# vbronetskyi/nclt-slam-project

Measured on AMD Instinct MI355X. Metric: relocalization frames/sec @640x480, 10k-landmark DB; Hamming-match HBM GB/s, higher is better.
Workload: dtype u8; 1 GPU; 640x480 BGR frames, 10000-record landmark DB (640000 descriptors, rows=fixed64), global relocalization tick per frame: ORB(500) + whole-DB mutual Hamming scan + top-25 PnP-RANSAC(200); frames resident in HBM, every frame's 96-byte result record written to pinned host memory by the tick's last kernel; distinct_frames=32, preroll_steps=20, streams=4, records=10000, descriptors=640000, parallelism=frames sharded across ranks, database replicated, no collective

## Files before the change

nclt-slam-project_amd/csrc/reloc_ctx.hip:

```cpp
#include <stdarg.h>
#include <stdlib.h>

#include "reloc_internal.h"

static thread_local char g_err[512] = "";

void reloc_set_error(const char *fmt, ...)
{
    va_list ap;
    va_start(ap, fmt);
    vsnprintf(g_err, sizeof(g_err), fmt, ap);
    va_end(ap);
}

RELOC_API const char *reloc_last_error(void) { return g_err; }

RELOC_API int reloc_device_count(void)
{
    int n = 0;
    if (hipGetDeviceCount(&n) != hipSuccess) return 0;
    return n;
}

template <typename T>
static int dalloc(T **p, int64_t count)
{
    HIP_TRY(hipMalloc((void **)p, (size_t)(count > 0 ? count : 1) * sizeof(T)));
    return 0;
}

static int ctx_alloc(reloc_ctx *c)
{
    int rc = 0;
    const int64_t mf = c->max_feat;
    int64_t pyr = 0;
    for (int l = 0; l < NLEV; ++l) {
        double s = pow(RELOC_ORB_SCALE_FACTOR, (double)l);
        int64_t w = (int64_t)(c->max_w / s) + 2, h = (int64_t)(c->max_h / s) + 2;
        pyr += ((w + 63) / 64 * 64) * h + 256;
    }
    c->pyr_bytes = pyr;
    rc |= dalloc(&c->pyr, pyr);
    rc |= dalloc(&c->blur, pyr);
    rc |= dalloc(&c->nms, pyr);
    rc |= dalloc(&c->rz_tab, (int64_t)NLEV * 2 * 2 * (c->max_w > c->max_h ? c->max_w : c->max_h));
    rc |= dalloc((char **)&c->pyr_tiles, (int64_t)((c->max_w + 15) / 16) * ((c->max_h + 15) / 16) * 128);
    rc |= dalloc(&c->hist, NLEV * 256);
    rc |= dalloc(&c->cand_cnt, NLEV);
    rc |= dalloc(&c->cand_key, (int64_t)NLEV * RELOC_ORB_STAGE1_CAP);
    rc |= dalloc(&c->cand_resp, (int64_t)NLEV * RELOC_ORB_STAGE1_CAP);
    rc |= dalloc(&c->kp_cnt, NLEV);
    rc |= dalloc(&c->kp_key, (int64_t)NLEV * RELOC_ORB_STAGE1_CAP);
    rc |= dalloc(&c->kp_resp, (int64_t)NLEV * RELOC_ORB_STAGE1_CAP);
    rc |= dalloc(&c->f_xy, mf * 2);
    rc |= dalloc(&c->f_size, mf);
    rc |= dalloc(&c->f_angle, mf);
    rc |= dalloc(&c->f_resp, mf);
    rc |= dalloc(&c->f_oct, mf);
    rc |= dalloc(&c->f_desc, mf * 32);
    rc |= dalloc(&c->f_count, 1);
    rc |= dalloc(&c->frame_img, (int64_t)c->max_w * c->max_h * 3);
    rc |= dalloc((char **)&c->orb_const, 1024);
    rc |= dalloc(&c->dbg_cut, NLEV);
    rc |= dalloc(&c->cand_ids, MAX_CAND);
    rc |= dalloc(&c->cand_n, 1);
    rc |= dalloc(&c->m_qidx, (int64_t)MAX_CAND * MAX_REC_ROWS);
    rc |= dalloc(&c->m_tidx, (int64_t)MAX_CAND * MAX_REC_ROWS);
    rc |= dalloc(&c->m_dist, (int64_t)MAX_CAND * MAX_REC_ROWS);
    rc |= dalloc(&c->m_n, MAX_CAND);
    rc |= dalloc(&c->p_obj, (int64_t)MAX_CAND * MAX_REC_ROWS * 3);
    rc |= dalloc(&c->p_img, (int64_t)MAX_CAND * MAX_REC_ROWS * 2);
    rc |= dalloc(&c->p_Rt, (int64_t)MAX_CAND * MAX_HYP * 12);
    rc |= dalloc(&c->p_cnt, (int64_t)MAX_CAND * MAX_HYP);
    rc |= dalloc(&c->p_inl, (int64_t)MAX_CAND * MAX_REC_ROWS);
    rc |= dalloc(&c->p_out, MAX_CAND);
    rc |= dalloc(&c->tick_res, 1);
    if (hipHostMalloc((void **)&c->tick_res_host, sizeof(TickResult), hipHostMallocDefault) != hipSuccess) {
        reloc_set_error("hipHostMalloc(result record) failed");
        c->tick_res_host = nullptr;
        rc |= RELOC_E_HIP;
    } else memset(c->tick_res_host, 0, sizeof(TickResult));
    rc |= dalloc(&c->accum_res, 1);
    rc |= dalloc(&c->tick_flags, 4);
    rc |= dalloc(&c->scan_ticket, (8 * 8 + 1) * 32);
    if (rc == 0 && hipMemset(c->scan_ticket, 0, (8 * 8 + 1) * 32 * 4) != hipSuccess) rc = RELOC_E_HIP;
    return rc;
}

int g_reloc_live_contexts = 0;

RELOC_API reloc_ctx *reloc_create(int device, int max_w, int max_h, int max_feat)
{
    int n = 0;
    if (hipGetDeviceCount(&n) != hipSuccess || n <= 0) {
        reloc_set_error("no HIP device available (libreloc_hip has no CPU fallback)");
        return nullptr;
    }
    if (device < 0 || device >= n || max_w < 64 || max_h < 64 || max_feat < 64) {
        reloc_set_error("reloc_create: bad arguments (device %d of %d, %dx%d, max_feat %d)", device, n,
                        max_w, max_h, max_feat);
        return nullptr;
    }
    if (hipSetDevice(device) != hipSuccess) {
        reloc_set_error("hipSetDevice(%d) failed", device);
        return nullptr;
    }
    reloc_ctx *c = new reloc_ctx();
    __atomic_add_fetch(&g_reloc_live_contexts, 1, __ATOMIC_RELAXED);
    c->device = device;
    c->max_w = max_w;
    c->max_h = max_h;
    c->max_feat = max_feat;
    hipDeviceProp_t prop;
    if (hipGetDeviceProperties(&prop, device) == hipSuccess) c->num_cu = prop.multiProcessorCount;
    if (hipStreamCreateWithFlags(&c->own_stream, hipStreamNonBlocking) != hipSuccess ||
        hipEventCreate(&c->t0) != hipSuccess || hipEventCreate(&c->t1) != hipSuccess) {
        reloc_set_error("stream/event creation failed");
        __atomic_sub_fetch(&g_reloc_live_contexts, 1, __ATOMIC_RELAXED);
        delete c;
        return nullptr;
    }
    c->stream = c->own_stream;
    c->prm.nfeatures = 500;
    c->prm.max_candidates = RELOC_MAX_CANDIDATES;
    c->prm.min_matches = RELOC_MIN_MATCHES;
    c->prm.min_inliers = RELOC_MIN_INLIERS;
    c->prm.ransac_iterations = RELOC_RANSAC_ITERATIONS;
    c->prm.global_max_candidates = RELOC_GLOBAL_MAX_CANDIDATES;
    c->prm.global_min_inliers = RELOC_GLOBAL_MIN_INLIERS;
    c->prm.accum_min_kpts = RELOC_ACCUM_MIN_KPTS;
    c->prm.candidate_radius_m = RELOC_CANDIDATE_RADIUS_M;
    c->prm.heading_tol_deg = RELOC_HEADING_TOL_DEG;
    c->prm.reproj_max_px = RELOC_REPROJ_MAX_PX;
    c->prm.ransac_reproj_px = RELOC_RANSAC_REPROJ_PX;
    c->prm.ransac_confidence = RELOC_RANSAC_CONFIDENCE;
    c->prm.consistency_m = RELOC_CONSISTENCY_M;
    c->prm.global_reproj_max_px = RELOC_GLOBAL_REPROJ_MAX_PX;
    c->prm.accum_min_dist_m = RELOC_ACCUM_MIN_DIST_M;
    c->prm.accum_depth_min_m = RELOC_ACCUM_DEPTH_MIN_M;
    c->prm.accum_depth_max_m = RELOC_ACCUM_DEPTH_MAX_M;
    c->prm.gray_coeff_bits = RELOC_GRAY_DEFAULT_BITS;
    c->prm.reserved0 = 0;
    if (const char *dev = getenv("RELOC_DEV"); dev && dev[0] == '1' && dev[1] == 0) {
        if (const char *e = getenv("RELOC_SCAN_GENS")) c->scan_gens = atoi(e);
        if (const char *e = getenv("RELOC_LOCAL_TWO_STAGE")) c->local_two_stage = atoi(e) != 0;
    }
    if (ctx_alloc(c) != 0) {
        reloc_destroy(c);
        return nullptr;
    }
    return c;
}

RELOC_API void reloc_destroy(reloc_ctx *c)
{
    if (!c) return;
    (void)hipSetDevice(c->device);
    if (c->stream) (void)hipStreamSynchronize(c->stream);
    db_arrays_drop(c->db_share, c->db_desc, c->db_pts3d, c->db_kp2d, c->db_off, c->db_pose, c->db_xy_heading);
    void *ptrs[] = {c->pyr, c->blur, c->nms, c->rz_tab, c->pyr_tiles, c->hist, c->cand_cnt, c->cand_key, c->cand_resp,
                    c->kp_cnt, c->kp_key, c->kp_resp, c->f_xy, c->f_size, c->f_angle, c->f_resp, c->f_oct,
                    c->f_desc, c->f_count, c->frame_img, c->orb_const, c->dbg_cut, c->db_counts, c->topk_part, c->cand_ids, c->cand_n, c->m_qidx,
                    c->m_tidx, c->m_dist, c->m_n, c->p_obj, c->p_img, c->p_Rt, c->p_cnt, c->p_inl,
                    c->p_out, c->tick_res, c->accum_res, c->tick_flags, c->scan_ticket, c->clahe_plane, c->clahe_lut,
                    c->rect_xy };
    for (void *p : ptrs)
        if (p) (void)hipFree(p);
    if (c->tick_res_host) (void)hipHostFree(c->tick_res_host);
    {
        DbArena &a = c->db_slot[1 - c->db_sel];
        db_arrays_drop(a.share, a.desc, a.pts3d, a.kp2d, a.off, a.pose, a.xy_heading);
        if (a.counts) (void)hipFree(a.counts);
        if (a.topk_part) (void)hipFree(a.topk_part);
    }
    for (int i = 0; i < 8; ++i)
        if (c->scratch[i]) (void)hipFree(c->scratch[i]);
    for (int k = 0; k < RELOC_PROF_N; ++k)
        if (c->prof[k].init)
            for (int i = 0; i < RELOC_PROF_RING; ++i) {
                (void)hipEventDestroy(c->prof[k].a[i]);
                (void)hipEventDestroy(c->prof[k].b[i]);
            }
    if (c->t0) (void)hipEventDestroy(c->t0);
    if (c->t1) (void)hipEventDestroy(c->t1);
    if (c->own_stream) (void)hipStreamDestroy(c->own_stream);
    __atomic_sub_fetch(&g_reloc_live_contexts, 1, __ATOMIC_RELAXED);
    delete c;
}

RELOC_API int reloc_get_params(reloc_ctx *c, reloc_params *out)
{
    ARG_CHECK_CTX(c, out, "reloc_get_params");
    *out = c->prm;
    return RELOC_OK;
}

RELOC_API int reloc_set_params(reloc_ctx *c, const reloc_params *p)
{
    ARG_CHECK_CTX(c, p, "reloc_set_params");
// ... 181 lines not shown
```

nclt-slam-project_amd/csrc/reloc_orb.hip:

```cpp
#include <math.h>

#include "../../include/reloc_orb_pattern.h"
#include "reloc_internal.h"

typedef uint32_t u32;

constexpr int HARRIS_CHUNK = 1024;
static_assert(HARRIS_CHUNK == 1024, "k_harris reads one dword per thread");

struct OrbTable {
    OrbLevel lev[NLEV];
    int fast_tile_base[NLEV + 1];
    int blur_tile_base[NLEV + 1];
    int flat_base[NLEV + 1];
    int rz_off[NLEV][4];
};

__constant__ signed char c_pattern[RELOC_ORB_NTESTS * 4];
__constant__ int c_umax[16] = {15, 15, 15, 15, 14, 14, 14, 13, 13, 12, 11, 10, 9, 8, 6, 3};
__constant__ signed char c_ring_dx[16] = {0, 1, 2, 3, 3, 3, 2, 1, 0, -1, -2, -3, -3, -3, -2, -1};
__constant__ signed char c_ring_dy[16] = {3, 3, 2, 1, 0, -1, -2, -3, -3, -3, -2, -1, 0, 1, 2, 3};

__device__ __forceinline__ int find_level(const int *base, int id)
{
    int l = 0;
#pragma unroll
    for (int k = 1; k < NLEV; ++k) l += id >= base[k];
    return l;
}

__device__ __forceinline__ int reflect101(int p, int n)
{
    if (n == 1) return 0;
    while (p < 0 || p >= n) {
        if (p < 0) p = -p;
        if (p >= n) p = 2 * n - 2 - p;
    }
    return p;
}

__device__ __forceinline__ int gray_fixed(int b, int g, int r, int flags)
{
    const bool c15 = flags & RELOC_GRAY_FLAG_15BIT;
    const int cb = c15 ? RELOC_GRAY15_CB : RELOC_GRAY_CB, cg = c15 ? RELOC_GRAY15_CG : RELOC_GRAY_CG, cr = c15 ? RELOC_GRAY15_CR : RELOC_GRAY_CR;
    const int sh = c15 ? RELOC_GRAY15_SHIFT : RELOC_GRAY_SHIFT;
    return (b * cb + g * cg + r * cr + (1 << (sh - 1))) >> sh;
}
static inline int gray_flags(const reloc_ctx *ctx, int order)
{
    return (order & 1) | (ctx->prm.gray_coeff_bits == RELOC_GRAY15_SHIFT ? RELOC_GRAY_FLAG_15BIT : 0);
}
__global__ __launch_bounds__(256) void k_gray_plain(const uint8_t *__restrict__ src, int w, int h, int sstride, int order_rgb,
                                                    uint8_t *__restrict__ dst)
{
    const int x = blockIdx.x * 256 + threadIdx.x, y = blockIdx.y;
    if (x >= w) return;
    const uint8_t *s = src + (size_t)y * sstride + 3 * x;
    const int c0 = s[0], c1 = s[1], c2 = s[2];
    const int b = (order_rgb & 1) ? c2 : c0, r = (order_rgb & 1) ? c0 : c2;
    dst[(size_t)y * w + x] = (uint8_t)gray_fixed(b, c1, r, order_rgb);
}

#ifndef PYR_TW
#define PYR_TW 64
#define PYR_TH 32
#endif
constexpr int PT_W = PYR_TW, PT_H = PYR_TH;
struct PyrTile {
    uint16_t o[NLEV][4];
    uint16_t n[NLEV][4];
};
static_assert(sizeof(PyrTile) == 128, "PyrTile is read as 8 dwordx4");

struct PyrLds { int lev[NLEV]; int tabs; };

struct OrbFrame {
    const OrbTable *tab; const PyrTile *tiles; const int32_t *rz; const uint8_t *src;
    uint8_t *pyr, *nms, *blur; int32_t *hist, *cand_cnt; u32 *cand_key; float *cand_resp; int32_t *dbg_cut;
    int32_t *kp_cnt; u32 *kp_key; float *kp_resp; float *f_xy, *f_size, *f_angle, *f_resp; int32_t *f_oct; uint8_t *f_desc;
    int32_t *f_count;
};
struct OrbBatch { OrbFrame f[RELOC_BATCH_MAX]; };

template <int CH, bool ALIGNED>
__device__ __forceinline__ void pyr_fetch(const uint8_t *sp, int x4, int w, u32 (&d)[3])
{
    if (ALIGNED) {
        const u32 *s4 = reinterpret_cast<const u32 *>(sp);
        d[0] = s4[0];
        if (CH == 3) { d[1] = s4[1]; d[2] = s4[2]; }
    } else {
        d[0] = d[1] = d[2] = 0;
#pragma unroll
        for (int k = 0; k < 4 * CH; ++k)
            if (x4 + k / CH < w) d[k >> 2] |= (u32)sp[k] << (8 * (k & 3));
    }
}

template <int CH>
__device__ __forceinline__ u32 pyr_gray4(const u32 (&d)[3], int x4, int w, int order_rgb)
{
    if (CH == 1) return d[0];
    u32 out = 0;
#pragma unroll
    for (int k = 0; k < 4; ++k) {
        int c[3];
#pragma unroll
        for (int j = 0; j < 3; ++j) { const int bi = 3 * k + j; c[j] = (d[bi >> 2] >> (8 * (bi & 3))) & 0xFF; }
        const int b = (order_rgb & 1) ? c[2] : c[0], r = (order_rgb & 1) ? c[0] : c[2];
        const int g = gray_fixed(b, c[1], r, order_rgb);
        if (x4 + k < w) out |= (u32)g << (8 * k);
    }
    return out;
}

__device__ __forceinline__ void pyr_tab_index(const OrbTable *__restrict__ tab, const PyrTile &T, const int (&tbase)[NLEV + 1], int i,
                                              int &po, int &pc)
{
    int j = i, nw = 0, x0 = 0, y0 = 0, ox = 0, cx = 0, oy = 0, cy = 0;
#pragma unroll
    for (int k = 1; k < NLEV; ++k) {
        const bool m = i >= tbase[k];
        j = m ? i - tbase[k] : j;
        nw = m ? T.n[k][1] - T.n[k][0] : nw;
        x0 = m ? (int)T.n[k][0] : x0;
        y0 = m ? (int)T.n[k][2] : y0;
        ox = m ? tab->rz_off[k][0] : ox;
        cx = m ? tab->rz_off[k][1] : cx;
        oy = m ? tab->rz_off[k][2] : oy;
        cy = m ? tab->rz_off[k][3] : cy;
    }
    const bool isx = j < nw;
    const int p = isx ? x0 + j : y0 + j - nw;
    po = (isx ? ox : oy) + p;
    pc = (isx ? cx : cy) + p;
}

__device__ __forceinline__ int pyr_div(int q, float inv) { return (int)(((float)q + 0.5f) * inv); }

template <int CH, bool ALIGNED, int PYR_BS>
__device__ __forceinline__ void pyramid_body(const OrbTable *__restrict__ tab, const PyrTile *__restrict__ tiles,
                                                 const int32_t *__restrict__ rz, const uint8_t *__restrict__ src, int w, int h,
                                                 int sstride, int order_rgb, uint8_t *__restrict__ pyr, PyrLds lds,
                                                 int32_t *__restrict__ hist, int32_t *__restrict__ cand_cnt)
{
    extern __shared__ u32 s_pyr[];
    const int tid = threadIdx.x;
    if (blockIdx.x == 0) {
        for (int i = tid; i < NLEV * 256; i += PYR_BS) hist[i] = 0;
        if (tid < NLEV) cand_cnt[tid] = 0;
    }
    const PyrTile &T = tiles[blockIdx.x];
    uint8_t *const base = reinterpret_cast<uint8_t *>(s_pyr);
    u32 *const tabs = s_pyr + (lds.tabs >> 2);
    int tbase[NLEV + 1];
    tbase[1] = 0;
#pragma unroll
    for (int l = 1; l < NLEV; ++l) tbase[l + 1] = tbase[l] + (T.n[l][1] - T.n[l][0]) + (T.n[l][3] - T.n[l][2]);
    constexpr int TAB_IT = 1024 / PYR_BS, L0_IT = 1536 / PYR_BS;
    u32 tv[TAB_IT][2];
#pragma unroll
    for (int it = 0; it < TAB_IT; ++it) {
        const int i = tid + it * PYR_BS;
        tv[it][0] = tv[it][1] = 0;
        if (i < tbase[NLEV]) {
            int po, pc;
            pyr_tab_index(tab, T, tbase, i, po, pc);
            tv[it][0] = (u32)rz[po];
            tv[it][1] = (u32)rz[pc];
        }
    }
    const int x00 = T.n[0][0], y00 = T.n[0][2], qpr0 = (T.n[0][1] - x00 + 3) >> 2, nq0 = qpr0 * (T.n[0][3] - y00);
    const float inv0 = 1.0f / (float)(qpr0 > 0 ? qpr0 : 1);
    u32 fv[L0_IT][3];
#pragma unroll
    for (int it = 0; it < L0_IT; ++it) {
        const int q = tid + it * PYR_BS;
        if (q < nq0) {
            const int ry = pyr_div(q, inv0), x4 = x00 + (q - ry * qpr0) * 4;
            pyr_fetch<CH, ALIGNED>(src + (size_t)(y00 + ry) * sstride + CH * x4, x4, w, fv[it]);
        }
    }
#pragma unroll
    for (int it = 0; it < TAB_IT; ++it) {
        const int i = tid + it * PYR_BS;
        if (i < tbase[NLEV]) tabs[i] = tv[it][0] | tv[it][1] << 16;
    }
#pragma unroll
    for (int it = 0; it < L0_IT; ++it) {
        const int q = tid + it * PYR_BS;
        if (q < nq0) {
            const int ry = pyr_div(q, inv0), x4 = x00 + (q - ry * qpr0) * 4;
            reinterpret_cast<u32 *>(base + lds.lev[0])[q] = pyr_gray4<CH>(fv[it], x4, w, order_rgb);
        }
    }
    for (int q = tid + L0_IT * PYR_BS; q < nq0; q += PYR_BS) {
        const int ry = pyr_div(q, inv0), x4 = x00 + (q - ry * qpr0) * 4;
        u32 d[3];
        pyr_fetch<CH, ALIGNED>(src + (size_t)(y00 + ry) * sstride + CH * x4, x4, w, d);
        reinterpret_cast<u32 *>(base + lds.lev[0])[q] = pyr_gray4<CH>(d, x4, w, order_rgb);
    }
    for (int i = tid + TAB_IT * PYR_BS; i < tbase[NLEV]; i += PYR_BS) {
        int po, pc;
        pyr_tab_index(tab, T, tbase, i, po, pc);
        tabs[i] = (u32)rz[po] | (u32)rz[pc] << 16;
    }
    __syncthreads();
#pragma unroll
    for (int l = 0; l + 1 < NLEV; ++l) {
        const int sw = tab->lev[l].w, sh = tab->lev[l].h;
        const uint8_t *cur = base + lds.lev[l];
        u32 *nxt = reinterpret_cast<u32 *>(base + lds.lev[l + 1]);
        const int nx0 = T.n[l][0], ny0 = T.n[l][2], pitch = ((T.n[l][1] - nx0 + 3) >> 2) << 2;
        const int dx0 = T.n[l + 1][0], dx1 = T.n[l + 1][1], dh = T.n[l + 1][3] - T.n[l + 1][2];
        const int qpr = (dx1 - dx0 + 3) >> 2;
        const u32 *xt = tabs + tbase[l + 1], *yt = xt + (dx1 - dx0);
        const u32 one = 1u << RELOC_RESIZE_COEF_BITS;
        const float inv = 1.0f / (float)(qpr > 0 ? qpr : 1);
        for (int q = tid; q < qpr * dh; q += PYR_BS) {
            const int ry = pyr_div(q, inv), rx4 = (q - ry * qpr) * 4;
            const u32 ye = yt[ry];
            const int sy0 = (int)(ye & 0xFFFF), sy1 = sy0 + 1 < sh ? sy0 + 1 : sh - 1;
            const u32 b = ye >> 16;
            const uint8_t *r0 = cur + (sy0 - ny0) * pitch - nx0, *r1 = cur + (sy1 - ny0) * pitch - nx0;
            u32 out = 0;
#pragma unroll
            for (int k = 0; k < 4; ++k) {
                if (dx0 + rx4 + k < dx1) {
                    const u32 xe = xt[rx4 + k];
                    const int k0 = (int)(xe & 0xFFFF), k1 = k0 + 1 < sw ? k0 + 1 : sw - 1;
                    const u32 a = xe >> 16;
                    const u32 h0 = (u32)r0[k0] * (one - a) + (u32)r0[k1] * a;
                    const u32 h1 = (u32)r1[k0] * (one - a) + (u32)r1[k1] * a;
                    const u32 v = h0 * (one - b) + h1 * b;
                    out |= ((v + (1u << 15)) >> 16) << (8 * k);
                }
            }
            nxt[q] = out;
        }
        __syncthreads();
    }
#pragma unroll
    for (int l = 0; l < NLEV; ++l) {
        const OrbLevel L = tab->lev[l];
        const uint8_t *cur = base + lds.lev[l];
        const int nx0 = T.n[l][0], ny0 = T.n[l][2], pitch = ((T.n[l][1] - nx0 + 3) >> 2) << 2;
        const int x0 = T.o[l][0], x1 = T.o[l][1], y0 = T.o[l][2], oh = T.o[l][3] - y0;
        const int qpr = (x1 - x0) >> 2;
        uint8_t *dst = pyr + L.off;
        const float inv = 1.0f / (float)(qpr > 0 ? qpr : 1);
        for (int q = tid; q < qpr * oh; q += PYR_BS) {
            const int ry = pyr_div(q, inv), x4 = x0 + (q - ry * qpr) * 4;
            u32 v = 0;
            if (x4 < L.w) {
                v = *reinterpret_cast<const u32 *>(cur + (y0 + ry - ny0) * pitch + (x4 - nx0));
                if (x4 + 4 > L.w) v &= 0xFFFFFFFFu >> (8 * (x4 + 4 - L.w));
            }
            *reinterpret_cast<u32 *>(dst + (size_t)(y0 + ry) * L.stride + x4) = v;
        }
    }
}
template <int CH, bool ALIGNED, int PYR_BS>
__global__ __launch_bounds__(PYR_BS) void k_pyramid(const OrbTable *__restrict__ tab, const PyrTile *__restrict__ tiles,
                                                 const int32_t *__restrict__ rz, const uint8_t *__restrict__ src, int w, int h,
                                                 int sstride, int order_rgb, uint8_t *__restrict__ pyr, PyrLds lds,
                                                 int32_t *__restrict__ hist, int32_t *__restrict__ cand_cnt)
{
    RELOC_SMALL_KERNEL_PRIO();
    pyramid_body<CH, ALIGNED, PYR_BS>(tab, tiles, rz, src, w, h, sstride, order_rgb, pyr, lds, hist, cand_cnt);
}
template <int CH, bool ALIGNED, int PYR_BS>
__global__ __launch_bounds__(PYR_BS) void k_pyramid_batch(OrbBatch b, int w, int h, int sstride, int order_rgb, PyrLds lds)
{
    RELOC_SMALL_KERNEL_PRIO();
    const OrbFrame &F = b.f[blockIdx.y];
    pyramid_body<CH, ALIGNED, PYR_BS>(F.tab, F.tiles, F.rz, F.src, w, h, sstride, order_rgb, F.pyr, lds, F.hist, F.cand_cnt);
}


template <bool REFLECT>
__device__ __forceinline__ u32 halo_dword(const uint8_t *__restrict__ row, int gx, int w)
{
    if (gx >= 0 && gx + 4 <= w) return *reinterpret_cast<const u32 *>(row + gx);
    u32 v = 0;
#pragma unroll
    for (int k = 0; k < 4; ++k) {
        const int x = REFLECT ? reflect101(gx + k, w) : min(max(gx + k, 0), w - 1);
        v |= (u32)row[x] << (8 * k);
    }
    return v;
}

constexpr int BT_W = 64, BT_H = 16;
constexpr int BT_P = BT_W / 4 + 2;
static_assert(BT_W == 64 && BT_H == 16, "blur7_tile maps 256 lanes to 16 rows x 16 dwords");
__device__ __forceinline__ void blur7_tile(const OrbTable *__restrict__ tab, const uint8_t *__restrict__ pyr,
                                           uint8_t *__restrict__ blur, int bid)
{
    __shared__ u32 s_in[(BT_H + 6) * BT_P];
    __shared__ u32 s_h[(BT_H + 6) * BT_W / 2];
    const int l = find_level(tab->blur_tile_base, bid);
    const OrbLevel L = tab->lev[l];
    const int tile = bid - tab->blur_tile_base[l];
    const int tx = (L.w + BT_W - 1) / BT_W;
    const int x0 = (tile % tx) * BT_W, y0 = (tile / tx) * BT_H;
    const uint8_t *src = pyr + L.off;
    const int tid = threadIdx.x;
    const int r16 = tid >> 4, c16 = tid & 15;
    {
        const int e = tid - 6 * 16;
        const bool edge = e >= 0;
        const int rb = edge ? e >> 1 : BT_H + r16, db = edge ? (e & 1) * (BT_P - 1) : 1 + c16;
        const bool on = e < 2 * (BT_H + 6);
        const int gya = reflect101(y0 + r16 - 3, L.h), gyb = reflect101(y0 + rb - 3, L.h);
        const u32 va = halo_dword<true>(src + (size_t)gya * L.stride, x0 + 4 * c16, L.w);
        u32 vb = 0;
        if (on) vb = halo_dword<true>(src + (size_t)gyb * L.stride, x0 - 4 + 4 * db, L.w);
        s_in[r16 * BT_P + 1 + c16] = va;
        if (on) s_in[rb * BT_P + db] = vb;
    }
    __syncthreads();
    constexpr u32 W_LO = RELOC_BLUR_K0 | RELOC_BLUR_K1 << 8 | RELOC_BLUR_K2 << 16 | (u32)RELOC_BLUR_K3 << 24;
    constexpr u32 W_HI = RELOC_BLUR_K2 | RELOC_BLUR_K1 << 8 | RELOC_BLUR_K0 << 16;
    static_assert(RELOC_BLUR_K3 < 256 && 2 * (RELOC_BLUR_K0 + RELOC_BLUR_K1 + RELOC_BLUR_K2) + RELOC_BLUR_K3 <= 256, "blur taps");
#pragma unroll
    for (int t = 0; t < 2; ++t) {
        const int ry = t * BT_H + r16;
        if (ry < BT_H + 6) {
            const u32 *p = s_in + ry * BT_P + c16;
            const u32 d0 = p[0], d1 = p[1], d2 = p[2];
            u32 s[4];
#pragma unroll
            for (int k = 0; k < 4; ++k) {
                const u32 lo = k < 3 ? __builtin_amdgcn_alignbyte(d1, d0, 1 + k) : d1;
                const u32 hi = k < 3 ? __builtin_amdgcn_alignbyte(d2, d1, 1 + k) : d2;
                s[k] = __builtin_amdgcn_udot4(lo, W_LO, __builtin_amdgcn_udot4(hi, W_HI, 0u, false), false);
            }
            *reinterpret_cast<uint2 *>(s_h + ry * (BT_W / 2) + 2 * c16) = make_uint2(s[0] | s[1] << 16, s[2] | s[3] << 16);
        }
    }
    __syncthreads();
    {
        u32 c[7][4];
#pragma unroll
        for (int j = 0; j < 7; ++j) {
            const uint2 d = *reinterpret_cast<const uint2 *>(s_h + (r16 + j) * (BT_W / 2) + 2 * c16);
            c[j][0] = d.x & 0xFFFF; c[j][1] = d.x >> 16; c[j][2] = d.y & 0xFFFF; c[j][3] = d.y >> 16;
        }
        u32 out = 0;
#pragma unroll
        for (int k = 0; k < 4; ++k) {
            const u32 s = RELOC_BLUR_K0 * (c[0][k] + c[6][k]) + RELOC_BLUR_K1 * (c[1][k] + c[5][k]) +
                          RELOC_BLUR_K2 * (c[2][k] + c[4][k]) + RELOC_BLUR_K3 * c[3][k];
            out |= ((s + (1u << 15)) >> 16) << (8 * k);
        }
        const int gy = y0 + r16, gx = x0 + 4 * c16;
        if (gy < L.h && gx < L.stride) *reinterpret_cast<u32 *>(blur + L.off + (size_t)gy * L.stride + gx) = out;
    }
}

__device__ int fast_is_corner(const uint8_t *p, int stride, int thr)
{
    const int c = p[0];
    u32 bright = 0, dark = 0;
#pragma unroll
    for (int k = 0; k < 16; ++k) {
        const int v = (int)p[c_ring_dy[k] * stride + c_ring_dx[k]] - c;
        bright |= (u32)(v > thr) << k;
        dark |= (u32)(v < -thr) << k;
    }
    auto run9 = [](u32 m) {
        u32 x = m | (m << 16);
        u32 y = x & (x >> 1);
        y &= y >> 2;
        y &= y >> 4;
        y &= x >> 8;
        return (y & 0xFFFFu) != 0;
    };
    return run9(bright) ? 1 : (run9(dark) ? -1 : 0);
}

__device__ int fast_corner_score(const uint8_t *p, int stride, int thr, int sign)
{
    const int c = p[0];
    int v[16];
#pragma unroll
    for (int k = 0; k < 16; ++k) v[k] = sign * ((int)p[c_ring_dy[k] * stride + c_ring_dx[k]] - c);
    int m2[16], m4[16], best = 0;
#pragma unroll
    for (int k = 0; k < 16; ++k) m2[k] = min(v[k], v[(k + 1) & 15]);
#pragma unroll
    for (int k = 0; k < 16; ++k) m4[k] = min(m2[k], m2[(k + 2) & 15]);
#pragma unroll
    for (int k = 0; k < 16; ++k) {
        const int m8 = min(m4[k], m4[(k + 4) & 15]);
        const int m9 = min(m8, v[(k + 8) & 15]);
        best = max(best, m9);
    }
    return best > thr ? best - 1 : 0;
}

__device__ __forceinline__ bool fast_run9(u32 x)
{
// ... 541 lines not shown
    for (int it = 0; it < 4; ++it) {
        const signed char *t = c_pattern + 4 * (64 * it + lane);
        int val[2];
#pragma unroll
        for (int e = 0; e < 2; ++e) {
            const float px = (float)t[2 * e], py = (float)t[2 * e + 1];
            const float rx = __fsub_rn(__fmul_rn(px, cs), __fmul_rn(py, sn));
            const float ry = __fadd_rn(__fmul_rn(px, sn), __fmul_rn(py, cs));
            const int ix = (int)rintf(rx), iy = (int)rintf(ry);
            val[e] = bc[iy * L.stride + ix];
        }
        bits[it] = __ballot(val[0] < val[1]);
    }
    if (lane < 4) {
        const unsigned long long b = lane == 0 ? bits[0] : lane == 1 ? bits[1] : lane == 2 ? bits[2] : bits[3];
        reinterpret_cast<unsigned long long *>(f_desc + (size_t)g * 32)[lane] = b;
    }
    if (lane == 0) {
        f_xy[2 * g] = __fmul_rn((float)x, L.scale);
        f_xy[2 * g + 1] = __fmul_rn((float)y, L.scale);
        f_size[g] = __fmul_rn((float)RELOC_ORB_PATCH, L.scale);
        f_angle[g] = angle;
        f_resp[g] = kp_resp[(size_t)l * RELOC_ORB_STAGE1_CAP + i];
        f_oct[g] = l;
    }
}
__global__ __launch_bounds__(256) void k_describe(const OrbTable *__restrict__ tab, const uint8_t *__restrict__ pyr,
                                                  const uint8_t *__restrict__ blur, const int32_t *__restrict__ kp_cnt,
                                                  const u32 *__restrict__ kp_key, const float *__restrict__ kp_resp,
                                                  int max_feat, float *__restrict__ f_xy, float *__restrict__ f_size,
                                                  float *__restrict__ f_angle, float *__restrict__ f_resp,
                                                  int32_t *__restrict__ f_oct, uint8_t *__restrict__ f_desc,
                                                  int32_t *__restrict__ f_count)
{
    RELOC_SMALL_KERNEL_PRIO();
    describe_body(tab, pyr, blur, kp_cnt, kp_key, kp_resp, max_feat, f_xy, f_size, f_angle, f_resp, f_oct, f_desc, f_count);
}
__global__ __launch_bounds__(256) void k_describe_batch(OrbBatch b, int max_feat)
{
    RELOC_SMALL_KERNEL_PRIO();
    const OrbFrame &F = b.f[blockIdx.y];
    describe_body(F.tab, F.pyr, F.blur, F.kp_cnt, F.kp_key, F.kp_resp, max_feat, F.f_xy, F.f_size, F.f_angle, F.f_resp, F.f_oct, F.f_desc,
                  F.f_count);
}


static void resize_axis(int src_n, int dst_n, int32_t *ofs, int32_t *coef)
{
    const double scale = (double)src_n / (double)dst_n;
    for (int d = 0; d < dst_n; ++d) {
        double f = ((double)d + 0.5) * scale - 0.5;
        int s = (int)floor(f);
        double a = f - (double)s;
        if (s < 0) { s = 0; a = 0.0; }
        if (s >= src_n - 1) { s = src_n - 1; a = 0.0; }
        ofs[d] = s;
        coef[d] = (int32_t)lrint(a * (double)(1 << RELOC_RESIZE_COEF_BITS));
    }
}

static bool g_pattern_uploaded[64] = {};

int orb_prepare(reloc_ctx *ctx, int w, int h, int nfeatures)
{
    if (w > ctx->max_w || h > ctx->max_h) {
        reloc_set_error("frame %dx%d exceeds the ctx capacity %dx%d", w, h, ctx->max_w, ctx->max_h);
        return RELOC_E_CAPACITY;
    }
    if (ctx->orb_w == w && ctx->orb_h == h && ctx->orb_nfeat == nfeatures) return RELOC_OK;
    if (!g_pattern_uploaded[ctx->device & 63]) {
        HIP_TRY(hipMemcpyToSymbol(HIP_SYMBOL(c_pattern), RELOC_ORB_PATTERN, sizeof(RELOC_ORB_PATTERN)));
        g_pattern_uploaded[ctx->device & 63] = true;
    }
    OrbTable tab;
    memset(&tab, 0, sizeof(tab));
    int64_t off = 0;
    for (int l = 0; l < NLEV; ++l) {
        const float s = (float)pow(RELOC_ORB_SCALE_FACTOR, (double)l);
        OrbLevel &L = tab.lev[l];
        L.scale = s;
        L.w = (int)lrintf((float)w / s);
        L.h = (int)lrintf((float)h / s);
        L.stride = (L.w + 63) / 64 * 64;
        L.off = off;
        off += ((int64_t)L.stride * L.h + 255) / 256 * 256;
    }
    if (off > ctx->pyr_bytes) { reloc_set_error("pyramid arena too small"); return RELOC_E_CAPACITY; }
    {
        const float factor = (float)(1.0 / RELOC_ORB_SCALE_FACTOR);
        float nper = (float)(nfeatures * (1 - factor) / (1 - (float)pow((double)factor, (double)NLEV)));
        int sum = 0;
        for (int l = 0; l < NLEV - 1; ++l) {
            tab.lev[l].quota = (int)lrintf(nper);
            sum += tab.lev[l].quota;
            nper *= factor;
        }
        tab.lev[NLEV - 1].quota = nfeatures - sum > 0 ? nfeatures - sum : 0;
    }
    for (int l = 0; l < NLEV; ++l) {
        const OrbLevel &L = tab.lev[l];
        tab.fast_tile_base[l + 1] = tab.fast_tile_base[l] + (L.stride / FT) * ((L.h + FT - 1) / FT);
        tab.blur_tile_base[l + 1] = tab.blur_tile_base[l] + ((L.w + BT_W - 1) / BT_W) * ((L.h + BT_H - 1) / BT_H);
        tab.flat_base[l + 1] = tab.flat_base[l] + (int)(((int64_t)L.stride * L.h + HARRIS_CHUNK - 1) / HARRIS_CHUNK);
    }
    const int maxdim = ctx->max_w > ctx->max_h ? ctx->max_w : ctx->max_h;
    int32_t *host = (int32_t *)malloc(sizeof(int32_t) * (size_t)NLEV * 4 * maxdim);
    int pos = 0;
    for (int l = 1; l < NLEV; ++l) {
        const OrbLevel &S = tab.lev[l - 1], &D = tab.lev[l];
        tab.rz_off[l][0] = pos; tab.rz_off[l][1] = pos + D.w;
        resize_axis(S.w, D.w, host + pos, host + pos + D.w);
        pos += 2 * D.w;
        tab.rz_off[l][2] = pos; tab.rz_off[l][3] = pos + D.h;
        resize_axis(S.h, D.h, host + pos, host + pos + D.h);
        pos += 2 * D.h;
    }
    const int ntx = (w + PT_W - 1) / PT_W, nty = (h + PT_H - 1) / PT_H;
    PyrTile *tiles = (PyrTile *)calloc((size_t)ntx * nty, sizeof(PyrTile));
    int lds_lev[NLEV] = {}, lds_t = 0;
    for (int t = 0; t < ntx * nty; ++t) {
        const int tx = t % ntx, ty = t / ntx;
        PyrTile &T = tiles[t];
        int nx0 = 0, nx1 = 0, ny0 = 0, ny1 = 0;
        int tsum = 0;
        for (int l = NLEV - 1; l >= 0; --l) {
            const OrbLevel &L = tab.lev[l];
            const int quads = (l == 0 ? (L.w + 3) / 4 : L.stride / 4);
            const int ox0 = 4 * (int)((int64_t)tx * quads / ntx), ox1 = 4 * (int)((int64_t)(tx + 1) * quads / ntx);
            const int oy0 = (int)((int64_t)ty * L.h / nty), oy1 = (int)((int64_t)(ty + 1) * L.h / nty);
            T.o[l][0] = (uint16_t)ox0; T.o[l][1] = (uint16_t)ox1; T.o[l][2] = (uint16_t)oy0; T.o[l][3] = (uint16_t)oy1;
            int cx0 = ox0, cx1 = ox1 < L.w ? ox1 : L.w, cy0 = oy0, cy1 = oy1;
            const bool stores = ox0 < ox1 && oy0 < oy1;
            const bool own = cx0 < cx1 && cy0 < cy1, need = nx0 < nx1 && ny0 < ny1;
            if (need) {
                const int32_t *xo = host + tab.rz_off[l + 1][0], *yo = host + tab.rz_off[l + 1][2];
                int sx0 = xo[nx0], sx1 = xo[nx1 - 1] + 2, sy0 = yo[ny0], sy1 = yo[ny1 - 1] + 2;
                if (sx1 > L.w) sx1 = L.w;
                if (sy1 > L.h) sy1 = L.h;
                if (own) {
                    cx0 = cx0 < sx0 ? cx0 : sx0; cx1 = cx1 > sx1 ? cx1 : sx1;
                    cy0 = cy0 < sy0 ? cy0 : sy0; cy1 = cy1 > sy1 ? cy1 : sy1;
                } else {
                    cx0 = sx0; cx1 = sx1; cy0 = sy0; cy1 = sy1;
                }
            } else if (!own) {
                cx0 = cx1 = cy0 = cy1 = 0;
            }
            cx0 &= ~3;
            T.n[l][0] = (uint16_t)cx0; T.n[l][1] = (uint16_t)cx1; T.n[l][2] = (uint16_t)cy0; T.n[l][3] = (uint16_t)cy1;
            if (!stores) T.o[l][0] = T.o[l][1] = T.o[l][2] = T.o[l][3] = 0;
            nx0 = cx0; nx1 = cx1; ny0 = cy0; ny1 = cy1;
            const int bytes = ((cx1 - cx0 + 3) / 4 * 4) * (cy1 - cy0);
            lds_lev[l] = bytes > lds_lev[l] ? bytes : lds_lev[l];
            if (l >= 1) tsum += (cx1 - cx0) + (cy1 - cy0);
        }
        lds_t = tsum > lds_t ? tsum : lds_t;
    }
    ctx->pyr_ntiles = ntx * nty;
    {
        int o = 0;
        for (int l = 0; l < NLEV; ++l) { ctx->pyr_lds[l] = o; o += (lds_lev[l] + 15) / 16 * 16; }
        ctx->pyr_lds[NLEV] = o;
        ctx->pyr_lds_bytes = o + 4 * lds_t;
    }
    if (ctx->pyr_lds_bytes > 64 * 1024) { free(host); free(tiles); reloc_set_error("pyramid tile exceeds LDS"); return RELOC_E_CAPACITY; }
    hipError_t e0 = hipMemcpyAsync(ctx->pyr_tiles, tiles, sizeof(PyrTile) * (size_t)ntx * nty, hipMemcpyHostToDevice, ctx->stream);
    hipError_t e1 = hipMemcpyAsync(ctx->rz_tab, host, sizeof(int32_t) * (size_t)pos, hipMemcpyHostToDevice, ctx->stream);
    hipError_t e2 = hipMemcpyAsync(ctx->orb_const, &tab, sizeof(tab), hipMemcpyHostToDevice, ctx->stream);
    hipError_t e3 = hipStreamSynchronize(ctx->stream);
    free(host);
    free(tiles);
    HIP_TRY(e0); HIP_TRY(e1); HIP_TRY(e2); HIP_TRY(e3);
    memcpy(ctx->lev, tab.lev, sizeof(tab.lev));
    memcpy(ctx->orb_tab_host, &tab, sizeof(tab));
    ctx->orb_w = w; ctx->orb_h = h; ctx->orb_nfeat = nfeatures;
    return RELOC_OK;
}

struct ClaheGeom {
    int w, h;
    int tx, ty;
    int tw, th;
    int clip;
    float lut_scale;
    float inv_tw, inv_th;
};
struct ClaheFrames { const uint8_t *src[RELOC_BATCH_MAX]; uint8_t *lut[RELOC_BATCH_MAX]; uint8_t *dst[RELOC_BATCH_MAX]; };
#ifndef RELOC_CLAHE_LUT_BS
#define RELOC_CLAHE_LUT_BS 1024
#endif
constexpr int CLAHE_LUT_BS = RELOC_CLAHE_LUT_BS;
constexpr int CLAHE_MAX_TILES = RELOC_CLAHE_MAX_TILES;

static ClaheGeom clahe_geom(int w, int h, double clip_limit, int tx, int ty)
{
    ClaheGeom g;
    g.w = w; g.h = h; g.tx = tx; g.ty = ty;
    const bool divides = w % tx == 0 && h % ty == 0;
    g.tw = divides ? w / tx : (w + tx - w % tx) / tx;
    g.th = divides ? h / ty : (h + ty - h % ty) / ty;
    const int area = g.tw * g.th;
    if (clip_limit > 0.0) {
        const int c = (int)(clip_limit * area / 256);
        g.clip = c > 1 ? c : 1;
    } else {
        g.clip = 0;
    }
    g.lut_scale = 255.0f / (float)area;
    g.inv_tw = 1.0f / (float)g.tw;
    g.inv_th = 1.0f / (float)g.th;
    return g;
}

template <int CH>
__global__ __launch_bounds__(CLAHE_LUT_BS) void k_clahe_lut(ClaheFrames F, ClaheGeom g, int sstride, int flags)
{
    constexpr int NWAVE = CLAHE_LUT_BS / 64;
    __shared__ int s_hist[NWAVE][256];
    const int tid = threadIdx.x, wave = tid >> 6, lane = tid & 63;
    for (int i = tid; i < NWAVE * 256; i += CLAHE_LUT_BS) (&s_hist[0][0])[i] = 0;
    __syncthreads();
    const uint8_t *src = F.src[blockIdx.y];
    const int ti = blockIdx.x % g.tx, tj = blockIdx.x / g.tx;
    const int x0 = ti * g.tw, y0 = tj * g.th;
    for (int py = wave; py < g.th; py += NWAVE) {
        const int sy = y0 + py < g.h ? y0 + py : reflect101(y0 + py, g.h);
        const uint8_t *row = src + (size_t)sy * sstride;
        for (int px = lane; px < g.tw; px += 64) {
            const int sx = x0 + px < g.w ? x0 + px : reflect101(x0 + px, g.w);
            int v;
            if (CH == 1) {
                v = row[sx];
            } else {
                const uint8_t *p = row + 3 * sx;
                const int c0 = p[0], c1 = p[1], c2 = p[2];
                v = gray_fixed((flags & 1) ? c2 : c0, c1, (flags & 1) ? c0 : c2, flags);
            }
            atomicAdd(&s_hist[wave][v], 1);
        }
    }
    __syncthreads();
    if (wave != 0) return;
    int hb[4];
#pragma unroll
    for (int k = 0; k < 4; ++k) {
        int s = 0;
#pragma unroll
        for (int wv = 0; wv < NWAVE; ++wv) s += s_hist[wv][4 * lane + k];
        hb[k] = s;
    }
    if (g.clip > 0) {
        int clipped = 0;
#pragma unroll
        for (int k = 0; k < 4; ++k) {
            const int ex = hb[k] > g.clip ? hb[k] - g.clip : 0;
            clipped += ex;
            hb[k] -= ex;
        }
        clipped = wave_sum_i32(clipped);
        const int batch = clipped >> 8, residual = clipped & 255;
        const int step = residual ? (256 / residual > 1 ? 256 / residual : 1) : 1;
#pragma unroll
        for (int k = 0; k < 4; ++k) {
            const int bin = 4 * lane + k;
            hb[k] += batch + (residual && bin % step == 0 && bin / step < residual ? 1 : 0);
        }
    }
    int loc[4];
    loc[0] = hb[0];
#pragma unroll
    for (int k = 1; k < 4; ++k) loc[k] = loc[k - 1] + hb[k];
    int incl = loc[3];
#pragma unroll
    for (int off = 1; off < 64; off <<= 1) {
        const int t = __shfl_up(incl, off);
        if (lane >= off) incl += t;
    }
    const int excl = incl - loc[3];
    u32 out = 0;
#pragma unroll
    for (int k = 0; k < 4; ++k) {
        int v = __float2int_rn((float)(excl + loc[k]) * g.lut_scale);
        v = v < 0 ? 0 : (v > 255 ? 255 : v);
        out |= (u32)v << (8 * k);
    }
    reinterpret_cast<u32 *>(F.lut[blockIdx.y] + (size_t)blockIdx.x * 256)[lane] = out;
}

template <int CH, bool ALIGNED>
__global__ __launch_bounds__(256) void k_clahe_apply(ClaheFrames F, ClaheGeom g, int sstride, int flags, int dstride)
{
    const int quads = (g.w + 3) >> 2;
    const int q = blockIdx.x * 256 + threadIdx.x;
    if (q >= quads * g.h) return;
    const int y = q / quads, x4 = 4 * (q - y * quads);
    u32 d[3];
    pyr_fetch<CH, ALIGNED>(F.src[blockIdx.y] + (size_t)y * sstride + CH * x4, x4, g.w, d);
    const u32 gray4 = pyr_gray4<CH>(d, x4, g.w, flags);
    const float tyf = (float)y * g.inv_th - 0.5f;
    int ty1 = (int)floorf(tyf);
    const float ya = tyf - (float)ty1, ya1 = 1.0f - ya;
    const int ty2 = ty1 + 1 < g.ty - 1 ? ty1 + 1 : g.ty - 1;
    ty1 = ty1 > 0 ? ty1 : 0;
    const uint8_t *lut = F.lut[blockIdx.y];
    const uint8_t *L1 = lut + (size_t)ty1 * g.tx * 256, *L2 = lut + (size_t)ty2 * g.tx * 256;
    u32 out = 0;
#pragma unroll
    for (int k = 0; k < 4; ++k) {
        const int x = x4 + k;
        const float txf = (float)x * g.inv_tw - 0.5f;
        int tx1 = (int)floorf(txf);
        const float xa = txf - (float)tx1, xa1 = 1.0f - xa;
        const int tx2 = tx1 + 1 < g.tx - 1 ? tx1 + 1 : g.tx - 1;
        tx1 = tx1 > 0 ? tx1 : 0;
        const int v = (gray4 >> (8 * k)) & 0xFF;
        const float l11 = L1[tx1 * 256 + v], l12 = L1[tx2 * 256 + v], l21 = L2[tx1 * 256 + v], l22 = L2[tx2 * 256 + v];
        const float res = (l11 * xa1 + l12 * xa) * ya1 + (l21 * xa1 + l22 * xa) * ya;
        int r = __float2int_rn(res);
        r = r < 0 ? 0 : (r > 255 ? 255 : r);
        if (x < g.w) out |= (u32)r << (8 * k);
    }
    uint8_t *dst = F.dst[blockIdx.y] + (size_t)y * dstride + x4;
    if ((dstride & 3) == 0) {
// ... 521 lines not shown
```

Before: 7427 frames/s.

## Repack pyramid resize tables and use dot-product intrinsics for gray and bilinear

```diff
diff --git a/nclt-slam-project_amd/csrc/reloc_ctx.hip b/nclt-slam-project_amd/csrc/reloc_ctx.hip
--- a/nclt-slam-project_amd/csrc/reloc_ctx.hip
+++ b/nclt-slam-project_amd/csrc/reloc_ctx.hip
@@ -44,7 +44,7 @@
     rc |= dalloc(&c->blur, pyr);
     rc |= dalloc(&c->nms, pyr);
     rc |= dalloc(&c->rz_tab, (int64_t)NLEV * 2 * 2 * (c->max_w > c->max_h ? c->max_w : c->max_h));
-    rc |= dalloc((char **)&c->pyr_tiles, (int64_t)((c->max_w + 15) / 16) * ((c->max_h + 15) / 16) * 128);
+    rc |= dalloc((char **)&c->pyr_tiles, (int64_t)((c->max_w + 15) / 16) * ((c->max_h + 15) / 16) * 192);
     rc |= dalloc(&c->hist, NLEV * 256);
     rc |= dalloc(&c->cand_cnt, NLEV);
     rc |= dalloc(&c->cand_key, (int64_t)NLEV * RELOC_ORB_STAGE1_CAP);
diff --git a/nclt-slam-project_amd/csrc/reloc_orb.hip b/nclt-slam-project_amd/csrc/reloc_orb.hip
--- a/nclt-slam-project_amd/csrc/reloc_orb.hip
+++ b/nclt-slam-project_amd/csrc/reloc_orb.hip
@@ -69,8 +69,10 @@
 struct PyrTile {
     uint16_t o[NLEV][4];
     uint16_t n[NLEV][4];
+    float inv_n[NLEV];
+    float inv_o[NLEV];
 };
-static_assert(sizeof(PyrTile) == 128, "PyrTile is read as 8 dwordx4");
+static_assert(sizeof(PyrTile) == 192, "PyrTile is read as 12 dwordx4");
 
 struct PyrLds { int lev[NLEV]; int tabs; };
 
@@ -114,29 +116,43 @@
     return out;
 }
 
-__device__ __forceinline__ void pyr_tab_index(const OrbTable *__restrict__ tab, const PyrTile &T, const int (&tbase)[NLEV + 1], int i,
-                                              int &po, int &pc)
-{
-    int j = i, nw = 0, x0 = 0, y0 = 0, ox = 0, cx = 0, oy = 0, cy = 0;
-#pragma unroll
-    for (int k = 1; k < NLEV; ++k) {
-        const bool m = i >= tbase[k];
-        j = m ? i - tbase[k] : j;
-        nw = m ? T.n[k][1] - T.n[k][0] : nw;
-        x0 = m ? (int)T.n[k][0] : x0;
-        y0 = m ? (int)T.n[k][2] : y0;
-        ox = m ? tab->rz_off[k][0] : ox;
-        cx = m ? tab->rz_off[k][1] : cx;
-        oy = m ? tab->rz_off[k][2] : oy;
-        cy = m ? tab->rz_off[k][3] : cy;
-    }
-    const bool isx = j < nw;
-    const int p = isx ? x0 + j : y0 + j - nw;
-    po = (isx ? ox : oy) + p;
-    pc = (isx ? cx : cy) + p;
+struct GrayW { u32 lo, hi, rnd, sh; };
+__device__ __forceinline__ GrayW gray_weights(int flags)
+{
+    const bool c15 = flags & RELOC_GRAY_FLAG_15BIT, rgb = flags & 1;
+    const u32 cb = c15 ? RELOC_GRAY15_CB : RELOC_GRAY_CB, cg = c15 ? RELOC_GRAY15_CG : RELOC_GRAY_CG, cr = c15 ? RELOC_GRAY15_CR : RELOC_GRAY_CR;
+    const u32 c0 = rgb ? cr : cb, c2 = rgb ? cb : cr;
+    GrayW g;
+    g.lo = (c0 & 0xFF) | (cg & 0xFF) << 8 | (c2 & 0xFF) << 16;
+    g.hi = (c0 >> 8) | (cg >> 8) << 8 | (c2 >> 8) << 16;
+    g.sh = c15 ? RELOC_GRAY15_SHIFT : RELOC_GRAY_SHIFT;
+    g.rnd = 1u << (g.sh - 1);
+    return g;
+}
+template <int CH>
+__device__ __forceinline__ u32 pyr_gray4_dot(const u32 (&d)[3], const GrayW &g)
+{
+    if (CH == 1) return d[0];
+    const u32 p[3] = {d[0], __builtin_amdgcn_alignbyte(d[1], d[0], 3), __builtin_amdgcn_alignbyte(d[2], d[1], 2)};
+    u32 v[4];
+#pragma unroll
+    for (int k = 0; k < 3; ++k)
+        v[k] = ((__builtin_amdgcn_udot4(p[k], g.hi, 0u, false) << 8) + __builtin_amdgcn_udot4(p[k], g.lo, g.rnd, false)) >> g.sh;
+    v[3] = ((__builtin_amdgcn_udot4(d[2], g.hi << 8, 0u, false) << 8) + __builtin_amdgcn_udot4(d[2], g.lo << 8, g.rnd, false)) >> g.sh;
+    return v[0] | v[1] << 8 | v[2] << 16 | v[3] << 24;
 }
 
 __device__ __forceinline__ int pyr_div(int q, float inv) { return (int)(((float)q + 0.5f) * inv); }
+
+typedef unsigned short __attribute__((ext_vector_type(2))) pyr_u16x2;
+__device__ __forceinline__ u32 pyr_dot2(u32 lo, u32 hi, u32 w, u32 acc)
+{
+    const u32 p = lo | hi << 16;
+    return __builtin_amdgcn_udot2(__builtin_bit_cast(pyr_u16x2, p), __builtin_bit_cast(pyr_u16x2, w), acc, false);
+}
+
+__device__ __forceinline__ int pyr_tab_cols(const PyrTile &T, int l) { return (T.n[l][1] - T.n[l][0] + 3) & ~3; }
+__device__ __forceinline__ int pyr_tab_rows(const PyrTile &T, int l) { return (T.n[l][3] - T.n[l][2] + 1) & ~1; }
 
 template <int CH, bool ALIGNED, int PYR_BS>
 __device__ __forceinline__ void pyramid_body(const OrbTable *__restrict__ tab, const PyrTile *__restrict__ tiles,
@@ -152,26 +168,26 @@
     }
     const PyrTile &T = tiles[blockIdx.x];
     uint8_t *const base = reinterpret_cast<uint8_t *>(s_pyr);
-    u32 *const tabs = s_pyr + (lds.tabs >> 2);
+    uint2 *const tabs = reinterpret_cast<uint2 *>(s_pyr + (lds.tabs >> 2));
     int tbase[NLEV + 1];
     tbase[1] = 0;
 #pragma unroll
-    for (int l = 1; l < NLEV; ++l) tbase[l + 1] = tbase[l] + (T.n[l][1] - T.n[l][0]) + (T.n[l][3] - T.n[l][2]);
-    constexpr int TAB_IT = 1024 / PYR_BS, L0_IT = 1536 / PYR_BS;
-    u32 tv[TAB_IT][2];
-#pragma unroll
-    for (int it = 0; it < TAB_IT; ++it) {
-        const int i = tid + it * PYR_BS;
-        tv[it][0] = tv[it][1] = 0;
-        if (i < tbase[NLEV]) {
-            int po, pc;
-            pyr_tab_index(tab, T, tbase, i, po, pc);
-            tv[it][0] = (u32)rz[po];
-            tv[it][1] = (u32)rz[pc];
-        }
+    for (int l = 1; l < NLEV; ++l) tbase[l + 1] = tbase[l] + pyr_tab_cols(T, l) + pyr_tab_rows(T, l);
+    const uint2 *rz2 = reinterpret_cast<const uint2 *>(rz);
+    uint2 tv[NLEV];
+#pragma unroll
+    for (int l = 1; l < NLEV; ++l) {
+        const int nc = pyr_tab_cols(T, l), nw = T.n[l][1] - T.n[l][0], nh = T.n[l][3] - T.n[l][2];
+        const bool isx = tid < nc;
+        const int p = isx ? tid : tid - nc;
+        tv[l] = make_uint2(0u, 0u);
+        if (isx ? p < nw : p < nh)
+            tv[l] = rz2[isx ? (tab->rz_off[l][0] >> 1) + T.n[l][0] + p : (tab->rz_off[l][2] >> 1) + T.n[l][2] + p];
     }
     const int x00 = T.n[0][0], y00 = T.n[0][2], qpr0 = (T.n[0][1] - x00 + 3) >> 2, nq0 = qpr0 * (T.n[0][3] - y00);
-    const float inv0 = 1.0f / (float)(qpr0 > 0 ? qpr0 : 1);
+    const float inv0 = T.inv_n[0];
+    const GrayW gw = gray_weights(order_rgb);
+    constexpr int L0_IT = 1536 / PYR_BS;
     u32 fv[L0_IT][3];
 #pragma unroll
     for (int it = 0; it < L0_IT; ++it) {
@@ -181,62 +197,63 @@
             pyr_fetch<CH, ALIGNED>(src + (size_t)(y00 + ry) * sstride + CH * x4, x4, w, fv[it]);
         }
     }
-#pragma unroll
-    for (int it = 0; it < TAB_IT; ++it) {
-        const int i = tid + it * PYR_BS;
-        if (i < tbase[NLEV]) tabs[i] = tv[it][0] | tv[it][1] << 16;
-    }
+    auto tab_entry = [&](int l, int i, uint2 e) {
+        const int nc = pyr_tab_cols(T, l), spitch = pyr_tab_cols(T, l - 1);
+        const bool isx = i < nc;
+        const bool live = isx ? i < T.n[l][1] - T.n[l][0] : i - nc < T.n[l][3] - T.n[l][2];
+        const u32 off = isx ? e.x - T.n[l - 1][0] : (e.x - T.n[l - 1][2]) * (u32)spitch;
+        return make_uint2(live ? off : 0u, e.y);
+    };
+#pragma unroll
+    for (int l = 1; l < NLEV; ++l)
+        if (tid < tbase[l + 1] - tbase[l]) tabs[tbase[l] + tid] = tab_entry(l, tid, tv[l]);
 #pragma unroll
     for (int it = 0; it < L0_IT; ++it) {
         const int q = tid + it * PYR_BS;
-        if (q < nq0) {
-            const int ry = pyr_div(q, inv0), x4 = x00 + (q - ry * qpr0) * 4;
-            reinterpret_cast<u32 *>(base + lds.lev[0])[q] = pyr_gray4<CH>(fv[it], x4, w, order_rgb);
-        }
+        if (q < nq0) reinterpret_cast<u32 *>(base + lds.lev[0])[q] = pyr_gray4_dot<CH>(fv[it], gw);
     }
     for (int q = tid + L0_IT * PYR_BS; q < nq0; q += PYR_BS) {
         const int ry = pyr_div(q, inv0), x4 = x00 + (q - ry * qpr0) * 4;
         u32 d[3];
         pyr_fetch<CH, ALIGNED>(src + (size_t)(y00 + ry) * sstride + CH * x4, x4, w, d);
-        reinterpret_cast<u32 *>(base + lds.lev[0])[q] = pyr_gray4<CH>(d, x4, w, order_rgb);
-    }
-    for (int i = tid + TAB_IT * PYR_BS; i < tbase[NLEV]; i += PYR_BS) {
-        int po, pc;
-        pyr_tab_index(tab, T, tbase, i, po, pc);
-        tabs[i] = (u32)rz[po] | (u32)rz[pc] << 16;
-    }
+        reinterpret_cast<u32 *>(base + lds.lev[0])[q] = pyr_gray4_dot<CH>(d, gw);
+    }
+#pragma unroll
+    for (int l = 1; l < NLEV; ++l)
+        for (int i = tid + PYR_BS; i < tbase[l + 1] - tbase[l]; i += PYR_BS) {
+            const int nc = pyr_tab_cols(T, l);
+            const bool isx = i < nc;
+            const int p = isx ? i : i - nc;
+            uint2 e = make_uint2(0u, 0u);
+            if (isx ? p < T.n[l][1] - T.n[l][0] : p < T.n[l][3] - T.n[l][2])
+                e = rz2[isx ? (tab->rz_off[l][0] >> 1) + T.n[l][0] + p : (tab->rz_off[l][2] >> 1) + T.n[l][2] + p];
+            tabs[tbase[l] + i] = tab_entry(l, i, e);
+        }
     __syncthreads();
 #pragma unroll
     for (int l = 0; l + 1 < NLEV; ++l) {
-        const int sw = tab->lev[l].w, sh = tab->lev[l].h;
         const uint8_t *cur = base + lds.lev[l];
         u32 *nxt = reinterpret_cast<u32 *>(base + lds.lev[l + 1]);
-        const int nx0 = T.n[l][0], ny0 = T.n[l][2], pitch = ((T.n[l][1] - nx0 + 3) >> 2) << 2;
-        const int dx0 = T.n[l + 1][0], dx1 = T.n[l + 1][1], dh = T.n[l + 1][3] - T.n[l + 1][2];
-        const int qpr = (dx1 - dx0 + 3) >> 2;
-        const u32 *xt = tabs + tbase[l + 1], *yt = xt + (dx1 - dx0);
-        const u32 one = 1u << RELOC_RESIZE_COEF_BITS;
-        const float inv = 1.0f / (float)(qpr > 0 ? qpr : 1);
+        const int pitch = pyr_tab_cols(T, l);
+        const int dh = T.n[l + 1][3] - T.n[l + 1][2], qpr = pyr_tab_cols(T, l + 1) >> 2;
+        const uint4 *xt = reinterpret_cast<const uint4 *>(tabs + tbase[l + 1]);
+        const uint2 *yt = tabs + tbase[l + 1] + 4 * qpr;
+        const float inv = T.inv_n[l + 1];
         for (int q = tid; q < qpr * dh; q += PYR_BS) {
-            const int ry = pyr_div(q, inv), rx4 = (q - ry * qpr) * 4;
-            const u32 ye = yt[ry];
-            const int sy0 = (int)(ye & 0xFFFF), sy1 = sy0 + 1 < sh ? sy0 + 1 : sh - 1;
-            const u32 b = ye >> 16;
-            const uint8_t *r0 = cur + (sy0 - ny0) * pitch - nx0, *r1 = cur + (sy1 - ny0) * pitch - nx0;
-            u32 out = 0;
+            const int ry = pyr_div(q, inv), rq = q - ry * qpr;
+            const uint2 ye = yt[ry];
+            const uint4 xa = xt[2 * rq], xb = xt[2 * rq + 1];
+            const u32 xo[4] = {xa.x, xa.z, xb.x, xb.z}, xw[4] = {xa.y, xa.w, xb.y, xb.w};
+            const uint8_t *r0 = cur + ye.x;
+            u32 v[4];
 #pragma unroll
             for (int k = 0; k < 4; ++k) {
-                if (dx0 + rx4 + k < dx1) {
-                    const u32 xe = xt[rx4 + k];
-                    const int k0 = (int)(xe & 0xFFFF), k1 = k0 + 1 < sw ? k0 + 1 : sw - 1;
-                    const u32 a = xe >> 16;
-                    const u32 h0 = (u32)r0[k0] * (one - a) + (u32)r0[k1] * a;
-                    const u32 h1 = (u32)r1[k0] * (one - a) + (u32)r1[k1] * a;
-                    const u32 v = h0 * (one - b) + h1 * b;
-                    out |= ((v + (1u << 15)) >> 16) << (8 * k);
-                }
+                const uint8_t *p0 = r0 + xo[k], *p1 = p0 + pitch;
+                const u32 h0 = pyr_dot2(p0[0], p0[1], xw[k], 0u);
+                const u32 h1 = pyr_dot2(p1[0], p1[1], xw[k], 0u);
+                v[k] = pyr_dot2(h0, h1, ye.y, 1u << 15);
             }
-            nxt[q] = out;
+            nxt[q] = __builtin_amdgcn_perm(v[1], v[0], 0x0c0c0602u) | __builtin_amdgcn_perm(v[3], v[2], 0x06020c0cu);
         }
         __syncthreads();
     }
@@ -244,11 +261,11 @@
     for (int l = 0; l < NLEV; ++l) {
         const OrbLevel L = tab->lev[l];
         const uint8_t *cur = base + lds.lev[l];
-        const int nx0 = T.n[l][0], ny0 = T.n[l][2], pitch = ((T.n[l][1] - nx0 + 3) >> 2) << 2;
+        const int nx0 = T.n[l][0], ny0 = T.n[l][2], pitch = pyr_tab_cols(T, l);
         const int x0 = T.o[l][0], x1 = T.o[l][1], y0 = T.o[l][2], oh = T.o[l][3] - y0;
         const int qpr = (x1 - x0) >> 2;
         uint8_t *dst = pyr + L.off;
-        const float inv = 1.0f / (float)(qpr > 0 ? qpr : 1);
+        const float inv = T.inv_o[l];
         for (int q = tid; q < qpr * oh; q += PYR_BS) {
             const int ry = pyr_div(q, inv), x4 = x0 + (q - ry * qpr) * 4;
             u32 v = 0;
@@ -1096,7 +1113,10 @@
             nx0 = cx0; nx1 = cx1; ny0 = cy0; ny1 = cy1;
             const int bytes = ((cx1 - cx0 + 3) / 4 * 4) * (cy1 - cy0);
             lds_lev[l] = bytes > lds_lev[l] ? bytes : lds_lev[l];
-            if (l >= 1) tsum += (cx1 - cx0) + (cy1 - cy0);
+            if (l >= 1) tsum += (cx1 - cx0 + 3) / 4 * 4 + (cy1 - cy0 + 1) / 2 * 2;
+            const int qn = (cx1 - cx0 + 3) / 4, qo = (T.o[l][1] - T.o[l][0]) / 4;
+            T.inv_n[l] = 1.0f / (float)(qn > 0 ? qn : 1);
+            T.inv_o[l] = 1.0f / (float)(qo > 0 ? qo : 1);
         }
         lds_t = tsum > lds_t ? tsum : lds_t;
     }
@@ -1105,14 +1125,25 @@
         int o = 0;
         for (int l = 0; l < NLEV; ++l) { ctx->pyr_lds[l] = o; o += (lds_lev[l] + 15) / 16 * 16; }
         ctx->pyr_lds[NLEV] = o;
-        ctx->pyr_lds_bytes = o + 4 * lds_t;
-    }
-    if (ctx->pyr_lds_bytes > 64 * 1024) { free(host); free(tiles); reloc_set_error("pyramid tile exceeds LDS"); return RELOC_E_CAPACITY; }
+        ctx->pyr_lds_bytes = o + 8 * lds_t + 128;
+    }
+    int32_t *packed = (int32_t *)malloc(sizeof(int32_t) * (size_t)(pos > 0 ? pos : 1));
+    for (int l = 1; l < NLEV; ++l)
+        for (int ax = 0; ax < 2; ++ax) {
+            const int n = ax ? tab.lev[l].h : tab.lev[l].w, at = tab.rz_off[l][2 * ax];
+            for (int d = 0; d < n; ++d) {
+                const int32_t c = host[at + n + d];
+                packed[at + 2 * d] = host[at + d];
+                packed[at + 2 * d + 1] = ((1 << RELOC_RESIZE_COEF_BITS) - c) | c << 16;
+            }
+        }
+    if (ctx->pyr_lds_bytes > 64 * 1024) { free(host); free(packed); free(tiles); reloc_set_error("pyramid tile exceeds LDS"); return RELOC_E_CAPACITY; }
     hipError_t e0 = hipMemcpyAsync(ctx->pyr_tiles, tiles, sizeof(PyrTile) * (size_t)ntx * nty, hipMemcpyHostToDevice, ctx->stream);
-    hipError_t e1 = hipMemcpyAsync(ctx->rz_tab, host, sizeof(int32_t) * (size_t)pos, hipMemcpyHostToDevice, ctx->stream);
+    hipError_t e1 = hipMemcpyAsync(ctx->rz_tab, packed, sizeof(int32_t) * (size_t)pos, hipMemcpyHostToDevice, ctx->stream);
     hipError_t e2 = hipMemcpyAsync(ctx->orb_const, &tab, sizeof(tab), hipMemcpyHostToDevice, ctx->stream);
     hipError_t e3 = hipStreamSynchronize(ctx->stream);
     free(host);
+    free(packed);
     free(tiles);
     HIP_TRY(e0); HIP_TRY(e1); HIP_TRY(e2); HIP_TRY(e3);
     memcpy(ctx->lev, tab.lev, sizeof(tab.lev));
```

Result: no change. 7471 frames/s, median of 6 (+0.6%).
